# niessner/BundleFusion

Hardware: AMD Instinct MI355X
Metric: frames/sec end-to-end (SIFT+SBA+TSDF re-integrate), 640x480 @4mm (higher is better)
Workload: dtype f32

## Files before the change

bundlefusion_amd/capi.py:

```python
import ctypes as C
import os

import numpy as np

_HERE = os.path.dirname(os.path.abspath(__file__))
LIB_PATH = os.environ.get("BF_LIB_PATH") or os.path.join(_HERE, "lib", "libbf_hip.so")


class BFError(RuntimeError):
    pass


if not os.path.exists(LIB_PATH):
    raise ImportError(
        "bundlefusion_amd: %s is missing — build it with `python -c 'import __graft_entry__ as g; g.build()'` "
        "(there is no CPU fallback)" % LIB_PATH)

try:
    import torch
except ImportError:
    pass
lib = C.CDLL(LIB_PATH, mode=C.RTLD_GLOBAL)

SDF_BLOCK_SIZE = 8
# ... 171 lines not shown
    def set_external_alloc(self, enable=True):
        check(lib.bf_scene_set_external_alloc(self._h, int(enable)))

    def set_alloc_comm(self, comm, capacity_keys=1 << 17):
        check(lib.bf_scene_set_alloc_comm(self._h, comm._h if comm is not None else None, int(capacity_keys)))
        self._alloc_comm = comm

    def alloc_collect(self, cam_to_world, depth, cam, part, parts, keys, slots, count):
        d = self._data(depth, None)
        check(lib.bf_scene_alloc_collect(self._h, mat16(cam_to_world), C.byref(d), C.byref(cam), int(part), int(parts), C.c_void_p(keys.data_ptr()),
                                         C.c_void_p(slots.data_ptr()), C.c_void_p(count.data_ptr()), int(keys.numel())))

    def alloc_ingest(self, keys, count):
        check(lib.bf_scene_alloc_ingest(self._h, C.c_void_p(keys.data_ptr()), C.c_void_p(count.data_ptr()), int(keys.numel())))

    def alloc_place(self):
        check(lib.bf_scene_alloc_place(self._h))

    def alloc_sync(self):
        check(lib.bf_scene_alloc_sync(self._h))

    def set_arith(self, mode):
        check(lib.bf_scene_set_arith(self._h, {"exact": 0, "fast": 1}[mode]))

    def arith(self):
        m = C.c_int()
        check(lib.bf_scene_get_arith(self._h, C.byref(m)))
        return ("exact", "fast")[m.value]

    def reintegrate(self, old_cam_to_world, new_cam_to_world, depth, color, cam):
        data = self._data(depth, color)
        check(lib.bf_scene_reintegrate(self._h, mat16(old_cam_to_world), mat16(new_cam_to_world), C.byref(data), C.byref(cam)))

    def run_batch(self, ops, cam):
        assert 1 <= len(ops) <= SCENE_BATCH_MAX
        arr = (SceneBatchOp * len(ops))()
        for o, (kind, T0, T1, depth, color) in zip(arr, ops):
            o.kind = {"in": 0, "de": 1, "re": 2}.get(kind, kind)
            o.T0[:] = np.asarray(T0, np.float32).reshape(16).tolist()
            o.T1[:] = np.asarray(T1 if T1 is not None else T0, np.float32).reshape(16).tolist()
            o.data = self._data(depth, color)
            o.d_texels = None; o.wait_event = None
        check(lib.bf_scene_run_batch(self._h, arr, len(ops), C.byref(cam)))

    def garbage_collect(self):
        check(lib.bf_scene_garbage_collect(self._h))

    def compactify(self, cam_to_world, cam):
        check(lib.bf_scene_set_last_rigid_transform_and_compactify(self._h, mat16(cam_to_world), C.byref(cam)))

    def hash_data(self):
        hd = HashData()
        check(lib.bf_scene_get_hash_data(self._h, C.byref(hd)))
        return hd

    def hash_params(self):
        p = HashParams()
        check(lib.bf_scene_get_hash_params(self._h, C.byref(p)))
        return p

    def heap_free_count(self):
        v = C.c_uint32()
        check(lib.bf_scene_get_heap_free_count(self._h, C.byref(v)))
        return v.value

    def num_allocated_blocks(self):
        v = C.c_uint32()
        check(lib.bf_scene_get_num_allocated_blocks(self._h, C.byref(v)))
        return v.value

    def num_integrated_frames(self):
        v = C.c_uint32()
        check(lib.bf_scene_get_num_integrated_frames(self._h, C.byref(v)))
        return v.value

    def debug_hash(self):
# ... 1264 lines not shown
```

bundlefusion_amd/csrc/host.hip:

```cpp
#include <algorithm>
#include <atomic>
#include <cmath>
#include <condition_variable>
#include <cstring>
#include <deque>
#include <fstream>
#include <limits>
#include <list>
#include <mutex>
#include <thread>
#include <chrono>
#include <vector>

#include "../../include/bf_pipeline.h"
#include "../../include/bf_comm.h"
#include "../../include/bf_sensordata.h"
#include "bf_device.h"
#include "bf_internal.h"
#include "bf_se3.h"

using namespace bf;

#define BF_TRY(expr) do { int _rc = (expr); if (_rc != BF_OK) return _rc; } while (0)

// ... 1942 lines not shown
    struct VolCmd { int kind; bf_depth_camera_data data; const void* texels; float T0[16], T1[16]; int waitEv; };
    bool volBatching = true;
    std::vector<VolCmd> volPending;
    static const size_t MAX_QUEUE = 48;
    std::thread worker;
    std::mutex mu;
    std::condition_variable cvWork, cvIdle;
    std::deque<VolCmd> queue;
    bool stop = false, busy = false;
    int workerError = BF_OK;
    std::string workerMessage;
    uint32_t numIntegrate = 0, numDeIntegrate = 0;
    double volBusy = 0.0, volCommands = 0.0;
    double hostProfile[8] = {0, 0, 0, 0, 0, 0, 0, 0};
    struct TraceRec { uint32_t frame; double hEnq0, hEnq1, hDet0, hDet1, hWait0, hWait1, hBody1; hipEvent_t gDet, gChain0, gChain1; };
    std::string tracePath; std::vector<TraceRec> trace; hipEvent_t traceBase = nullptr; double traceBaseHost = 0.0;
    TraceRec* traceOf(uint32_t frame) { for (size_t i = trace.size(); i-- > 0;) if (trace[i].frame == frame) return &trace[i]; return nullptr; }
    bool timings = false;
    hipEvent_t ev[10] = {nullptr, nullptr, nullptr, nullptr, nullptr, nullptr, nullptr, nullptr, nullptr, nullptr};
    bf_frame_timing last;
};

namespace {

int volExecute(bf_pipeline* p, const bf_pipeline::VolCmd& c) {
    if (c.kind == 3) return bf_scene_garbage_collect(p->scene);
    if (c.waitEv >= 0) BF_TRY(bf_scene_wait_event(p->scene, p->evIngest[c.waitEv]));
    if (c.texels) BF_TRY(bf_scene_set_frame_texels(p->scene, c.texels));
    if (c.kind == 0) return bf_scene_integrate(p->scene, c.T0, &c.data, &p->cam, nullptr);
    if (c.kind == 1) return bf_scene_deintegrate(p->scene, c.T0, &c.data, &p->cam, nullptr);
    return bf_scene_reintegrate(p->scene, c.T0, c.T1, &c.data, &p->cam);
}

int volSubmitPending(bf_pipeline* p) {
    std::vector<bf_pipeline::VolCmd>& q = p->volPending;
    if (q.empty()) return BF_OK;
    bf_scene_batch_op ops[BF_SCENE_BATCH_MAX];
    const uint32_t n = (uint32_t)q.size();
    for (uint32_t k = 0; k < n; ++k) {
        const bf_pipeline::VolCmd& c = q[k];
        ops[k].kind = c.kind; ops[k].reserved = 0;
        memcpy(ops[k].T0, c.T0, 64); memcpy(ops[k].T1, c.kind == 2 ? c.T1 : c.T0, 64);
        ops[k].data = c.data; ops[k].d_texels = c.texels;
        ops[k].wait_event = c.waitEv >= 0 ? (void*)p->evIngest[c.waitEv] : nullptr;
    }
    q.clear();
    return bf_scene_run_batch(p->scene, ops, n, &p->cam);
}

int volHandle(bf_pipeline* p, const bf_pipeline::VolCmd& c) {
    if (!p->volBatching) return c.kind == 4 ? BF_OK : volExecute(p, c);
    if (c.kind <= 2) {
        p->volPending.push_back(c);
        return p->volPending.size() == BF_SCENE_BATCH_MAX ? volSubmitPending(p) : BF_OK;
    }
    BF_TRY(volSubmitPending(p));
    return c.kind == 3 ? bf_scene_garbage_collect(p->scene) : BF_OK;
}

void volWorker(bf_pipeline* p) {
    for (;;) {
        bf_pipeline::VolCmd c;
        {
            std::unique_lock<std::mutex> lk(p->mu);
            p->cvWork.wait(lk, [p] { return p->stop || !p->queue.empty(); });
            if (p->queue.empty()) return;
            c = p->queue.front(); p->queue.pop_front();
            p->busy = true;
        }
        const double tv = std::chrono::duration<double>(std::chrono::steady_clock::now().time_since_epoch()).count();
        const int rc = volHandle(p, c);
        const double dv = std::chrono::duration<double>(std::chrono::steady_clock::now().time_since_epoch()).count() - tv;
        {
            std::lock_guard<std::mutex> lk(p->mu);
            p->volBusy += dv; p->volCommands += 1.0;
            if (rc != BF_OK && p->workerError == BF_OK) { p->workerError = rc; p->workerMessage = bf_last_error(); }
            p->busy = false;
            p->cvIdle.notify_all();
        }
    }
}

int volPost(bf_pipeline* p, int kind, uint32_t frame, const float* T0, const float* T1, int waitEv) {
    bf_pipeline::VolCmd c;
    c.kind = kind; c.waitEv = waitEv;
    c.data.d_depthData = nullptr; c.data.d_colorData = nullptr;
    c.texels = nullptr;
    if (kind < 3) {
        BF_TRY(bf_image_manager_get_integrate_frame_gpu(p->im, frame, &c.data.d_depthData, &c.data.d_colorData));
        BF_TRY(bf_image_manager_get_integrate_frame_texels(p->im, frame, &c.texels));
// ... 666 lines not shown
```

bundlefusion_amd/csrc/tsdf.hip:

```cpp
#include <hip/hip_runtime.h>

#include <algorithm>
#include <cmath>
#include <cstdlib>
#include <cstring>
#include <strings.h>
#include <unordered_map>
#include <unordered_set>
#include <vector>

#include "bf_device.h"
#include "bf_internal.h"
#include "../../include/bf_comm.h"

using namespace bf;

namespace {

constexpr int BS = BF_SDF_BLOCK_SIZE;
constexpr int VOX = BS * BS * BS;
constexpr uint32_t NBINS = 256;
constexpr uint32_t BINCAP = 4096;
constexpr uint32_t OVCAP = 4096;
constexpr uint32_t TILE = 1024;
// ... 743 lines not shown
        lastFlag = ticket == gridDim.x - 1 ? 1u : 0u;
        if (lastFlag) __builtin_amdgcn_fence(__ATOMIC_ACQUIRE, "agent");
    }
    __syncthreads();
    if (!lastFlag) return;
    placeTail<LISTS>(d, f, fo, s, tailIn[0], tailIn[1], tailIn[2], tailIn[3]);
    if (threadIdx.x == 0) d.stats[ST_TICKET] = 0;
}

__global__ __launch_bounds__(256) void k_compact_count(Dev d) {
    __shared__ uint32_t wsum[4];
    __builtin_amdgcn_s_setprio(3);
    const uint32_t n = d.allocCount[0];
    const uint32_t numTiles = (n + TILE - 1) / TILE;
    for (uint32_t tile = blockIdx.x; tile < numTiles; tile += gridDim.x) {
        uint32_t c = 0;
#pragma unroll
        for (uint32_t k = 0; k < 4; ++k) {
            const uint32_t i = tile * TILE + threadIdx.x * 4 + k;
            if (i < n) c += d.allocList[i].ptr != BF_FREE_ENTRY ? 1u : 0u;
        }
        c = (uint32_t)wave_sum_i((int)c);
        if ((threadIdx.x & 63) == 0) wsum[threadIdx.x >> 6] = c;
        __syncthreads();
        if (threadIdx.x == 0) d.tileCounts[tile] = wsum[0] + wsum[1] + wsum[2] + wsum[3];
        __syncthreads();
    }
}

__global__ __launch_bounds__(256) void k_compact_scatter(Dev d) {
    __shared__ uint32_t wsum[4];
    __builtin_amdgcn_s_setprio(3);
    __shared__ uint32_t wscan[4];
    const uint32_t n = d.allocCount[0];
    const uint32_t numTiles = (n + TILE - 1) / TILE;
    const uint32_t lane = threadIdx.x & 63, wave = threadIdx.x >> 6;
    for (uint32_t tile = blockIdx.x; tile < numTiles; tile += gridDim.x) {
        uint32_t v = 0;
        for (uint32_t t = threadIdx.x; t < tile; t += blockDim.x) v += d.tileCounts[t];
        v = (uint32_t)wave_sum_i((int)v);
        if (lane == 0) wsum[wave] = v;
        __syncthreads();
        const uint32_t base = wsum[0] + wsum[1] + wsum[2] + wsum[3];
        __syncthreads();
        AllocRec recs[4];
        bool keep[4];
        uint32_t c = 0;
#pragma unroll
        for (uint32_t k = 0; k < 4; ++k) {
            const uint32_t i = tile * TILE + threadIdx.x * 4 + k;
            keep[k] = false;
            if (i < n) { recs[k] = d.allocList[i]; keep[k] = recs[k].ptr != BF_FREE_ENTRY; }
            c += keep[k] ? 1u : 0u;
        }
        uint32_t incl = c;
#pragma unroll
        for (int o = 1; o < 64; o <<= 1) { const uint32_t t = __shfl_up(incl, o, 64); if ((int)lane >= o) incl += t; }
        if (lane == 63) wscan[wave] = incl;
        __syncthreads();
        uint32_t woff = 0;
        for (uint32_t w = 0; w < wave; ++w) woff += wscan[w];
        const uint32_t tileTotal = wscan[0] + wscan[1] + wscan[2] + wscan[3];
        uint32_t pos = base + woff + incl - c;
#pragma unroll
        for (uint32_t k = 0; k < 4; ++k) if (keep[k]) d.allocListAlt[pos++] = recs[k];
        if (tile == numTiles - 1 && threadIdx.x == 0) d.tileCounts[numTiles] = base + tileTotal;
        __syncthreads();
    }
}

template <int MODE>
__global__ __launch_bounds__(256) void k_compact_append(Dev d, Frame f, Frame fo) {
    __shared__ uint32_t wscan[4];
    __shared__ uint32_t sbase;
    __builtin_amdgcn_s_setprio(3);
    listAppendTiles<MODE, 4>(d, f, fo, d.allocSnap[0], blockIdx.x, gridDim.x, wscan, &sbase);
}

__global__ void k_alloc_snapshot(Dev d) { d.allocSnap[0] = d.allocCount[0]; d.compactCount[0] = 0; d.compactCount[1] = 0; }

__global__ void k_list_commit(Dev d) {
    const uint32_t n = d.allocCount[0];
    const uint32_t numTiles = (n + TILE - 1) / TILE;
    if (numTiles > 0) d.allocCount[0] = d.tileCounts[numTiles];
}

template <bool DEINT, class FR>
BF_DEV void voxelApply(const FR& f, float sdf, uchar4 cc, float& vSdf, float& vW, uint32_t& vC) {
    const float c0 = (float)cc.x, c1 = (float)cc.y, c2 = (float)cc.z;
    const float oSdf = vSdf, oW = vW;
    const uint32_t oC = vC;
    const float o0 = (float)(oC & 0xFF), o1 = (float)((oC >> 8) & 0xFF), o2 = (float)((oC >> 16) & 0xFF);
    float nSdf, nW;
    uint32_t nC;
    if (!DEINT) {
        float r0, r1, r2;
        if (oW == 0.0f) { r0 = c0; r1 = c1; r2 = c2; }
        else { r0 = 0.2f * c0 + 0.8f * o0; r1 = 0.2f * c1 + 0.8f * o1; r2 = 0.2f * c2 + 0.8f * o2; }
        r0 = fmaxf(0.0f, fminf(__builtin_rintf(r0), 254.5f));
        r1 = fmaxf(0.0f, fminf(__builtin_rintf(r1), 254.5f));
        r2 = fmaxf(0.0f, fminf(__builtin_rintf(r2), 254.5f));
        nC = (uint32_t)(int)r0 | ((uint32_t)(int)r1 << 8) | ((uint32_t)(int)r2 << 16) | 0xFF000000u;
        nSdf = (sdf * 1.0f + oSdf * oW) / (1.0f + oW);
        nW = fminf(f.weightMax, 1.0f + oW);
    } else {
        float r0 = (o0 * oW - c0 * 1.0f) / (oW - 1.0f);
        float r1 = (o1 * oW - c1 * 1.0f) / (oW - 1.0f);
        float r2 = (o2 * oW - c2 * 1.0f) / (oW - 1.0f);
        r0 = fmaxf(0.0f, fminf(roundf(r0), 254.5f));
        r1 = fmaxf(0.0f, fminf(roundf(r1), 254.5f));
        r2 = fmaxf(0.0f, fminf(roundf(r2), 254.5f));
        nC = (uint32_t)(int)r0 | ((uint32_t)(int)r1 << 8) | ((uint32_t)(int)r2 << 16) | 0xFF000000u;
        nSdf = (oSdf * oW - sdf * 1.0f) / (oW - 1.0f);
        nW = fmaxf(0.0f, oW - 1.0f);
        if (nW <= 0.001f) { nSdf = 0.0f; nC = 0u; nW = 0.0f; }
    }
    vSdf = nSdf; vW = nW; vC = nC;
}
// ... 513 lines not shown
                h4[(size_t)i * 2] = h4[(size_t)next * 2];
                h4[(size_t)i * 2 + 1] = h4[(size_t)next * 2 + 1];
                h4[(size_t)next * 2] = make_uint4(0, 0, 0, (uint32_t)BF_FREE_ENTRY);
                h4[(size_t)next * 2 + 1] = make_uint4(0, 0, 0, 0);
            } else {
                h4[(size_t)i * 2] = make_uint4(0, 0, 0, (uint32_t)BF_FREE_ENTRY);
                h4[(size_t)i * 2 + 1] = make_uint4(0, 0, 0, 0);
            }
            return c.ptr;
        }
    }
    const uint32_t last = hp + BF_HASH_BUCKET_SIZE - 1;
    bf_hash_entry c = d.hash[last];
    uint32_t prev = last;
    uint32_t i = (last + c.offset) % total;
    for (uint32_t it = 0; it < f.maxChain; ++it) {
        c = d.hash[i];
        if (c.pos[0] == b.x && c.pos[1] == b.y && c.pos[2] == b.z && c.ptr != BF_FREE_ENTRY) {
            h4[(size_t)i * 2] = make_uint4(0, 0, 0, (uint32_t)BF_FREE_ENTRY);
            h4[(size_t)i * 2 + 1] = make_uint4(0, 0, 0, 0);
            d.hash[prev].offset = c.offset;
            return c.ptr;
        }
        if (c.offset == 0) return BF_FREE_ENTRY;
        prev = i;
        i = (last + c.offset) % total;
    }
    return BF_FREE_ENTRY;
}

__global__ __launch_bounds__(1024) void k_gc_delete(Dev d, Frame f) {
    __shared__ SortLds s;
    __shared__ uint32_t scratch[16];
    const uint32_t bin = blockIdx.x;
    const uint32_t n = min(d.binCount[bin], BINCAP);
    if (n == 0) return;
    loadBinSorted(s, d.bins + (size_t)bin * BINCAP, n);
    const uint32_t base = binPrefix(d.binCount, bin, scratch);
    const uint32_t heapC = d.heapCounter[0];
    for (uint32_t idx = threadIdx.x; idx < n; idx += blockDim.x) {
        const uint32_t h = s.bucket[idx];
        if (idx > 0 && s.bucket[idx - 1] == h) continue;
        for (uint32_t k = idx; k < n && s.bucket[k] == h; ++k) {
            const int32_t ptr = deleteEntry(d, f, unpackKey(s.key[k]), h);
            d.allocList[s.aux[k]].ptr = BF_FREE_ENTRY;
            if (ptr == BF_FREE_ENTRY) { atomicOr(&d.stats[ST_ERROR], (uint32_t)ERR_GC_MISSING); s.aux[k] = 0xFFFFFFFFu; continue; }
            d.heap[heapC + 1u + base + k] = (uint32_t)ptr / (uint32_t)VOX;
            s.aux[k] = (uint32_t)ptr;
        }
    }
    __syncthreads();
    for (uint32_t k = 0; k < n; ++k) {
        const uint32_t ptr = s.aux[k];
        if (ptr == 0xFFFFFFFFu) continue;
        uint4* v4 = reinterpret_cast<uint4*>(d.vox + (size_t)ptr);
        for (uint32_t t = threadIdx.x; t < (uint32_t)(VOX * 12 / 16); t += blockDim.x) v4[t] = make_uint4(0, 0, 0, 0);
    }
}

__global__ __launch_bounds__(256) void k_gc_finish(Dev d) {
    __shared__ uint32_t scratch[16];
    const uint32_t D = binPrefix(d.binCount, NBINS, scratch);
    if (threadIdx.x == 0) d.heapCounter[0] += D;
    __syncthreads();
    for (uint32_t b = threadIdx.x; b < NBINS; b += blockDim.x) d.binCount[b] = 0;
}

}

struct bf_scene {
    bf_hash_params params;
    bf_depth_camera_params cam;
    bool haveCam = false;
    Dev d{};
    hipStream_t stream = nullptr;
    uint32_t numIntegrated = 0;
    uint32_t dedupeSize = 0;
    uint32_t gridCompact = 0, gridUpdateCol = 0, gridUpdateColPlain = 0;
    bool forceExactDiv = false;
    bool externalAlloc = false;
    bf_comm* allocComm = nullptr;
    uint32_t allocCap = 0;
    uint8_t *d_allocSend = nullptr, *d_allocRecv = nullptr; uint32_t* d_allocSlots = nullptr;
    uint8_t *d_batchSend = nullptr, *d_batchRecv = nullptr;
    int arith = BF_TSDF_ARITH_FAST;
    int cvtRne = -1;
    uint2* texel[8] = {}; size_t texelPixels = 0;
    int32_t* d_hashDecision = nullptr;
    uint32_t shardLo = 0, shardHi = 0xFFFFFFFFu;
    uint32_t opsTimed = 0;
    uint32_t imagesTimed = 0;
    bool overlap = false;
    hipStream_t prep = nullptr;
    static constexpr int NBMAX = 8;
    int NB = 4;
    bf_hash_entry* cbuf[NBMAX] = {}; uint32_t* csrc[NBMAX] = {}; int32_t* ccnt[NBMAX] = {};
    int cur = 0;
// ... 419 lines not shown
        auto update = [&](const Dev& dd, int accumulate) {
            if (s->cvtRne) hipLaunchKernelGGL((k_update_batch_apx<true>), dim3(s->gridUpdateCol), dim3(256), s->updateLds, s->stream, dd, ac, ua, accumulate);
            else hipLaunchKernelGGL((k_update_batch_apx<false>), dim3(s->gridUpdateCol), dim3(256), s->updateLds, s->stream, dd, ac, ua, accumulate);
        };
        if (s->verifyPath) {
            BF_TRY_RC(verifyBuffers(s));
            hipLaunchKernelGGL(k_verify_copy, dim3(s->gridUpdateCol), dim3(256), 0, s->stream, dv, s->vshadow[0], s->vshadow[1]);
        }
        update(dv, acc);
        if (s->verifyPath) {
            for (int q = 0; q < 2; ++q) { Dev dq = dv; dq.vox = s->vshadow[q]; update(dq, 0); }
            hipLaunchKernelGGL(k_verify_compare, dim3(s->gridUpdateCol), dim3(256), 0, s->stream, dv, s->vshadow[0], s->vshadow[1], s->vlog, s->vseq++, n, s->gridUpdateCol * 4u);
        }
    } else {
        BatchUpdColArgs ua;
        memset(&ua, 0, sizeof ua);
        ua.nOps = n;
        for (uint32_t k = 0; k < n; ++k) {
            ua.op[k].in = makeUpdPose(fin[k]); ua.op[k].de = makeUpdPose(fde[k]);
            ua.op[k].depth = ops[k].data.d_depthData; ua.op[k].color = reinterpret_cast<const uchar4*>(ops[k].data.d_colorData);
        }
        hipLaunchKernelGGL(k_update_batch_col, dim3(s->gridUpdateCol), dim3(256), 0, s->stream, dv, makeUpdCam(fl), ua, acc, s->forceExactDiv ? 1 : 0);
    }
    if (ev) BF_HIP_TRY(hipEventRecord(ev->second, s->stream));
    if (s->overlap) { BF_HIP_TRY(hipEventRecord(s->evUpd[b], s->stream)); s->updRecorded[b] = true; }
    BF_HIP_TRY(hipGetLastError());
    useBuf(s, b);
    s->compactStale = true;
    s->gcMask = (ops[n - 1].kind == 1 ? 2u : 1u) << (2u * (n - 1));
    for (uint32_t k = 0; k < n; ++k) s->numIntegrated += ops[k].kind == 0 ? 1u : ops[k].kind == 1 ? (uint32_t)-1 : 0u;
    return BF_OK;
}

int checkCall(bf_scene* s, const float* T, const bf_depth_camera_data* data, const bf_depth_camera_params* cam,
              const uint32_t* d_bitMask) {
    BF_REQUIRE(s && T && data && cam, "null argument");
    BF_REQUIRE(data->d_depthData, "d_depthData is null");
    BF_REQUIRE(d_bitMask == nullptr, "chunk streaming (d_bitMask) is not supported: it is disabled for BundleFusion");
    BF_REQUIRE(cam->m_imageWidth > 0 && cam->m_imageHeight > 0, "empty image");
    return BF_OK;
}

}

extern "C" {

int bf_scene_create(const bf_hash_params* p, bf_scene** out) {
    BF_REQUIRE(p && out, "null argument");
    BF_REQUIRE(p->m_hashNumBuckets > 0 && p->m_numSDFBlocks > 0, "empty hash / heap");
    BF_REQUIRE(p->m_hashBucketSize == BF_HASH_BUCKET_SIZE, "m_hashBucketSize must be 4 (HASH_BUCKET_SIZE)");
    BF_REQUIRE(p->m_SDFBlockSize == BF_SDF_BLOCK_SIZE, "m_SDFBlockSize must be 8 (SDF_BLOCK_SIZE)");
    BF_REQUIRE((uint64_t)p->m_hashNumBuckets * BF_HASH_BUCKET_SIZE < 0x7FFFFFFFull, "hash too large for 32-bit slot indices");
    BF_REQUIRE((uint64_t)p->m_numSDFBlocks * VOX < 0x7FFFFFFFull, "too many SDF blocks for the reference's int ptr");
    int ndev = 0;
    if (hipGetDeviceCount(&ndev) != hipSuccess || ndev == 0) { set_error("no HIP device visible"); return BF_ERR_NO_DEVICE; }
    bf_scene* s = new bf_scene();
    s->params = *p;
    const size_t numEntries = (size_t)p->m_hashNumBuckets * BF_HASH_BUCKET_SIZE;
    const size_t N = p->m_numSDFBlocks;
    uint32_t ds = 1u << 16;
    while (ds < 2u * NBINS * BINCAP && ds < 4u * N) ds <<= 1;
    s->dedupeSize = ds;
    int rc = BF_OK;
#define A(ptr, cnt) if (rc == BF_OK) rc = devAlloc(s, &(ptr), (cnt))
    A(s->d.hash, numEntries);
    A(s->d.heap, N);
// ... 228 lines not shown
    int rc = checkCall(s, T, data, cam, d_bitMask);
    if (rc) return rc;
    s->cam = *cam; s->haveCam = true;
    setLastRigidTransform(s, T);
    const Frame f = makeFrame(s);
    if ((rc = runOperator(s, 1, f, f, data))) return rc;
    s->numIntegrated--;
    return BF_OK;
}

int bf_scene_set_shard(bf_scene* s, uint32_t rank, uint32_t world) {
    BF_REQUIRE(s && world >= 1 && rank < world, "bad shard");
    BF_REQUIRE(s->numIntegrated == 0, "set the shard before the first integration");
    const uint64_t nb = s->params.m_hashNumBuckets;
    s->shardLo = (uint32_t)(nb * rank / world);
    s->shardHi = (uint32_t)(nb * (rank + 1) / world);
    return BF_OK;
}

int bf_scene_reintegrate(bf_scene* s, const float oldT[16], const float newT[16], const bf_depth_camera_data* data,
                         const bf_depth_camera_params* cam) {
    int rc = checkCall(s, newT, data, cam, nullptr);
    if (rc) return rc;
    BF_REQUIRE(oldT, "null argument");
    s->cam = *cam; s->haveCam = true;
    setLastRigidTransform(s, oldT);
    const Frame fo = makeFrame(s);
    setLastRigidTransform(s, newT);
    const Frame f = makeFrame(s);
    return runOperator(s, 2, f, fo, data);
}

int bf_scene_run_batch(bf_scene* s, const bf_scene_batch_op* ops, uint32_t n, const bf_depth_camera_params* cam) {
    BF_REQUIRE(s && ops && cam, "null argument");
    BF_REQUIRE(n >= 1 && n <= BF_SCENE_BATCH_MAX, "1 .. BF_SCENE_BATCH_MAX operators per batch");
    BF_REQUIRE(cam->m_imageWidth > 0 && cam->m_imageHeight > 0, "empty image");
    for (uint32_t k = 0; k < n; ++k) {
        BF_REQUIRE(ops[k].kind >= 0 && ops[k].kind <= 2, "unknown operator kind");
        BF_REQUIRE(ops[k].data.d_depthData, "d_depthData is null");
    }
    s->cam = *cam; s->haveCam = true;
    return runBatch(s, ops, n);
}

int bf_scene_set_last_rigid_transform_and_compactify(bf_scene* s, const float T[16], const bf_depth_camera_params* cam) {
    BF_REQUIRE(s && T && cam, "null argument");
    s->cam = *cam; s->haveCam = true;
    setLastRigidTransform(s, T);
    BF_TRY_RC(beginExclusive(s));
    BF_TRY_RC(launchCompactify(s));
    return endExclusive(s);
}

int bf_scene_garbage_collect(bf_scene* s) {
    BF_REQUIRE(s, "null scene");
    if (!s->haveCam) return BF_OK;
    BF_TRY_RC(beginExclusive(s));
    uint32_t needMask = 0;
    if (s->compactStale) { if (s->gcMask) needMask = s->gcMask; else BF_TRY_RC(launchCompactify(s)); }
    const Frame f = makeFrame(s);
    hipLaunchKernelGGL(k_gc_identify, dim3(4096), dim3(256), 0, s->stream, s->d, f, needMask);
    hipLaunchKernelGGL(k_gc_delete, dim3(NBINS), dim3(1024), 0, s->stream, s->d, f);
    hipLaunchKernelGGL(k_gc_finish, dim3(1), dim3(256), 0, s->stream, s->d);
    hipLaunchKernelGGL(k_compact_count, dim3(s->gridCompact), dim3(256), 0, s->stream, s->d);
    hipLaunchKernelGGL(k_compact_scatter, dim3(s->gridCompact), dim3(256), 0, s->stream, s->d);
    hipLaunchKernelGGL(k_list_commit, dim3(1), dim3(1), 0, s->stream, s->d);
    std::swap(s->d.allocList, s->d.allocListAlt);
    BF_HIP_TRY(hipGetLastError());
    s->compactStale = true; s->gcMask = 0;
    return endExclusive(s);
}

int bf_scene_get_hash_data(bf_scene* s, bf_hash_data* out) {
    BF_REQUIRE(s && out, "null argument");
    BF_TRY_RC(refreshStaleList(s));
    BF_TRY_RC(syncAll(s));
    out->d_heap = s->d.heap;
    out->d_heapCounter = s->d.heapCounter;
    out->d_hashDecision = s->d_hashDecision;
    out->d_hashDecisionPrefix = nullptr;
    out->d_hash = s->d.hash;
    out->d_hashCompactified = s->d.compact;
    out->d_hashCompactifiedCounter = s->d.compactCount;
    out->d_SDFBlocks = s->d.vox;
    out->d_hashBucketMutex = nullptr;
    return BF_OK;
}

static int checkDeviceErrors(bf_scene* s) {
    uint32_t stats[ST_COUNT];
    BF_HIP_TRY(hipMemcpyAsync(stats, s->d.stats, sizeof stats, hipMemcpyDeviceToHost, s->stream));
    BF_HIP_TRY(hipStreamSynchronize(s->stream));
    if (stats[ST_ERROR]) { set_error("TSDF scratch capacity exceeded during an earlier operator (error bits 0x%x: 1 bin, 2 de-dup set, 4 overflow list, 8 GC, 16 block list)", stats[ST_ERROR]); return BF_ERR_CAPACITY; }
    return BF_OK;
}

int bf_scene_get_hash_params(bf_scene* s, bf_hash_params* out) {
    BF_REQUIRE(s && out, "null argument");
    BF_TRY_RC(refreshStaleList(s));
    BF_TRY_RC(syncAll(s));
    int32_t n = 0;
    BF_HIP_TRY(hipMemcpyAsync(&n, s->d.compactCount, 4, hipMemcpyDeviceToHost, s->stream));
    BF_HIP_TRY(hipStreamSynchronize(s->stream));
// ... 151 lines not shown
```

include/bf_hip.h:

```cpp
#ifndef BF_HIP_H
#define BF_HIP_H

#include <stddef.h>
#include <stdint.h>

#ifdef __cplusplus
extern "C" {
#endif

#define BF_API __attribute__((visibility("default")))

typedef enum bf_status {
    BF_OK = 0,
    BF_ERR_INVALID_ARG = -1,
    BF_ERR_HIP = -2,
    BF_ERR_NO_DEVICE = -3,
    BF_ERR_CAPACITY = -4,
    BF_ERR_STATE = -5,
    BF_ERR_NOT_ON_DEVICE = -6
} bf_status;

BF_API const char* bf_last_error(void);
BF_API const char* bf_version(void);
BF_API int bf_device_count(void);
// ... 78 lines not shown
                              const bf_depth_camera_data* data,
                              const bf_depth_camera_params* cam, const uint32_t* d_bitMask);
BF_API int bf_scene_deintegrate(bf_scene* s, const float cam_to_world[16],
                                const bf_depth_camera_data* data,
                                const bf_depth_camera_params* cam, const uint32_t* d_bitMask);
BF_API int bf_scene_set_overlap(bf_scene* s, int enable);
BF_API int bf_scene_wait_event(bf_scene* s, void* hip_event);
BF_API int bf_scene_set_shard(bf_scene* s, uint32_t rank, uint32_t world);
BF_API int bf_scene_set_external_alloc(bf_scene* s, int enable);
BF_API int bf_scene_alloc_collect(bf_scene* s, const float cam_to_world[16], const bf_depth_camera_data* data, const bf_depth_camera_params* cam,
                                  uint32_t part, uint32_t parts, uint64_t* d_keys, uint32_t* d_slots, uint32_t* d_count, uint32_t capacity);
BF_API int bf_scene_alloc_ingest(bf_scene* s, const uint64_t* d_keys, const uint32_t* d_count, uint32_t capacity);
BF_API int bf_scene_alloc_place(bf_scene* s);
BF_API int bf_scene_alloc_sync(bf_scene* s);
#define BF_TSDF_ARITH_EXACT 0
#define BF_TSDF_ARITH_FAST 1
BF_API int bf_scene_set_arith(bf_scene* s, int mode);
BF_API int bf_scene_set_frame_texels(bf_scene* s, const void* d_texels);
BF_API int bf_image_interleave_texels(void* d_texels, const float* d_depth, const uint8_t* d_colorRGBX, uint32_t numPixels, void* hip_stream);
BF_API int bf_scene_get_arith(bf_scene* s, int* mode);
BF_API int bf_scene_reintegrate(bf_scene* s, const float old_cam_to_world[16], const float new_cam_to_world[16],
                                const bf_depth_camera_data* data, const bf_depth_camera_params* cam);
#define BF_SCENE_BATCH_MAX 12
typedef struct bf_scene_batch_op {
    int32_t kind;
    int32_t reserved;
    float T0[16], T1[16];
    bf_depth_camera_data data;
    const void* d_texels;
    void* wait_event;
} bf_scene_batch_op;
BF_API int bf_scene_run_batch(bf_scene* s, const bf_scene_batch_op* ops, uint32_t n, const bf_depth_camera_params* cam);
BF_API int bf_scene_garbage_collect(bf_scene* s);
BF_API int bf_scene_set_last_rigid_transform_and_compactify(
    bf_scene* s, const float cam_to_world[16], const bf_depth_camera_params* cam);
BF_API int bf_scene_set_last_rigid_transform(bf_scene* s, const float cam_to_world[16]);
BF_API int bf_scene_get_hash_data(bf_scene* s, bf_hash_data* out);
BF_API int bf_scene_get_hash_params(bf_scene* s, bf_hash_params* out);
BF_API int bf_scene_get_heap_free_count(bf_scene* s, uint32_t* out);
BF_API int bf_scene_get_num_integrated_frames(bf_scene* s, uint32_t* out);
BF_API int bf_scene_debug_hash(bf_scene* s, uint32_t out[6]);
BF_API int bf_scene_debug_find_blocks(bf_scene* s, const int32_t* d_pos, uint32_t n, int32_t* d_ptr_out);
BF_API int bf_scene_get_num_allocated_blocks(bf_scene* s, uint32_t* out);
BF_API int bf_scene_kernel_timing(bf_scene* s, int enable);
BF_API int bf_scene_kernel_timing_read(bf_scene* s, uint32_t* count, float* total_ms);
BF_API int bf_scene_kernel_timing_occupied(bf_scene* s, uint64_t* sumOccupiedBlocks, uint32_t* numOps);
BF_API int bf_scene_kernel_timing_images(bf_scene* s, uint32_t* numImages);
BF_API int bf_scene_kernel_timing_blocks(bf_scene* s, uint64_t* sumOperatorBlocks, uint64_t* visitedPlain, uint64_t* visitedFused, uint32_t* numOps);



typedef struct bf_cached_frame {
    float* d_depthDownsampled;
    float* d_cameraposDownsampled;
    float* d_intensityDownsampled;
    float* d_intensityDerivsDownsampled;
    uint8_t* d_normalsDownsampledUCHAR4;
    float* d_normalsDownsampled;
} bf_cached_frame;

typedef struct bf_cache bf_cache;

BF_API int bf_cache_create(uint32_t widthDepthInput, uint32_t heightDepthInput, uint32_t widthDownSampled,
                           uint32_t heightDownSampled, uint32_t maxNumImages, const float inputIntrinsics[16],
                           float colorDownSigma, float depthDownSigmaD, float depthDownSigmaR, bf_cache** out);
BF_API int bf_cache_destroy(bf_cache* c);
// ... 275 lines not shown
```

include/bundlefusion/bundlefusion.hpp:

```cpp
#pragma once
#include <algorithm>
#include <array>
#include <cstdint>
#include <cstdio>
#include <cmath>
#include <cstring>
#include <fstream>
#include <iostream>
#include <limits>
#include <mutex>
#include <stdexcept>
#include <string>
#include <utility>
#include <vector>

#include "../bf_pipeline.h"
#include "../bf_sensordata.h"

namespace bundlefusion {

struct mat4f {
    float m[16];
    static mat4f identity() { mat4f r; for (int i = 0; i < 16; ++i) r.m[i] = (i % 5 == 0) ? 1.0f : 0.0f; return r; }
    float& operator()(int r, int c) { return m[r * 4 + c]; }
// ... 645 lines not shown
    bf_depth_camera_data d;
};

class CUDASceneRepHashSDF {
public:
    explicit CUDASceneRepHashSDF(const HashParams& params) { check(bf_scene_create(&params, &m_h)); }
    ~CUDASceneRepHashSDF() { try { flush(); } catch (...) {} bf_scene_destroy(m_h); }
    CUDASceneRepHashSDF(const CUDASceneRepHashSDF&) = delete;
    static HashParams parametersFromGlobalAppState(const GlobalAppState& gas) {
        HashParams p;
        std::memset(&p, 0, sizeof p);
        const mat4f I = mat4f::identity();
        std::memcpy(p.m_rigidTransform, I.m, 64); std::memcpy(p.m_rigidTransformInverse, I.m, 64);
        p.m_hashNumBuckets = gas.s_hashNumBuckets; p.m_hashBucketSize = 4; p.m_hashMaxCollisionLinkedListSize = gas.s_hashMaxCollisionLinkedListSize;
        p.m_SDFBlockSize = 8; p.m_numSDFBlocks = gas.s_hashNumSDFBlocks; p.m_virtualVoxelSize = gas.s_SDFVoxelSize;
        p.m_maxIntegrationDistance = gas.s_SDFMaxIntegrationDistance; p.m_truncation = gas.s_SDFTruncation; p.m_truncScale = gas.s_SDFTruncationScale;
        p.m_integrationWeightSample = gas.s_SDFIntegrationWeightSample; p.m_integrationWeightMax = gas.s_SDFIntegrationWeightMax;
        for (int i = 0; i < 3; ++i) { p.m_streamingVoxelExtents[i] = gas.s_streamingVoxelExtents[i]; p.m_streamingGridDimensions[i] = gas.s_streamingGridDimensions[i]; p.m_streamingMinGridPos[i] = gas.s_streamingMinGridPos[i]; }
        p.m_streamingInitialChunkListSize = gas.s_streamingInitialChunkListSize;
        return p;
    }
    void integrate(const mat4f& lastRigidTransform, const DepthCameraData& data, const DepthCameraParams& params, unsigned int* d_bitMask) {
        if (!m_deferred || d_bitMask) { flush(); check(bf_scene_integrate(m_h, lastRigidTransform.m, &data.d, &params, d_bitMask)); return; }
        if (!m_pending.empty() && m_pending.back().kind == 1 && m_pending.back().data.d_depthData == data.d.d_depthData && m_pending.back().data.d_colorData == data.d.d_colorData && m_lastWasDe) {
            m_pending.back().kind = 2; std::memcpy(m_pending.back().T1, lastRigidTransform.m, 64); m_lastWasDe = false;
        } else push(0, lastRigidTransform, data);
        m_cam = params;
    }
    void deIntegrate(const mat4f& lastRigidTransform, const DepthCameraData& data, const DepthCameraParams& params, unsigned int* d_bitMask) {
        if (!m_deferred || d_bitMask) { flush(); check(bf_scene_deintegrate(m_h, lastRigidTransform.m, &data.d, &params, d_bitMask)); return; }
        push(1, lastRigidTransform, data); m_lastWasDe = true;
        m_cam = params;
    }
    void garbageCollect() { flush(); check(bf_scene_garbage_collect(m_h)); }
    void reset() { m_pending.clear(); check(bf_scene_reset(m_h)); }
    void setLastRigidTransformAndCompactify(const mat4f& lastRigidTransform, const DepthCameraParams& params) {
        flush(); check(bf_scene_set_last_rigid_transform_and_compactify(m_h, lastRigidTransform.m, &params));
    }
    void setLastRigidTransform(const mat4f& lastRigidTransform) { flush(); check(bf_scene_set_last_rigid_transform(m_h, lastRigidTransform.m)); }
    const mat4f getLastRigidTransform() { const HashParams p = getHashParams(); mat4f m; std::memcpy(m.m, p.m_rigidTransform, 64); return m; }
    void debugHash() {
        flush();
        uint32_t v[6]; check(bf_scene_debug_hash(m_h, v));
        std::printf("number of occupied entries: %u\nfree heap: %u\nduplicate keys: %u\nallocated and free: %u\nleaked blocks: %u\ndropped: %u\n", v[0], v[1], v[2], v[3], v[4], v[5]);
    }
    HashDataStruct getHashData() { flush(); HashDataStruct d; check(bf_scene_get_hash_data(m_h, &d)); return d; }
    HashParams getHashParams() { flush(); HashParams p; check(bf_scene_get_hash_params(m_h, &p)); return p; }
    unsigned int getHeapFreeCount() { flush(); uint32_t n; check(bf_scene_get_heap_free_count(m_h, &n)); return n; }
    unsigned int getNumIntegratedFrames() { flush(); uint32_t n; check(bf_scene_get_num_integrated_frames(m_h, &n)); return n; }
    bf_scene* handle() const { return m_h; }

    void setDeferredBatching(bool enable) { flush(); m_deferred = enable; }
    void flush() {
        if (m_pending.empty()) return;
        std::vector<bf_scene_batch_op> ops; ops.swap(m_pending);
        m_lastWasDe = false;
        check(bf_scene_run_batch(m_h, ops.data(), (uint32_t)ops.size(), &m_cam));
    }
private:
    void push(int kind, const mat4f& T, const DepthCameraData& data) {
        if (m_pending.size() == BF_SCENE_BATCH_MAX) flush();
        bf_scene_batch_op o; std::memset(&o, 0, sizeof o);
        o.kind = kind; std::memcpy(o.T0, T.m, 64); std::memcpy(o.T1, T.m, 64); o.data = data.d;
        m_pending.push_back(o); m_lastWasDe = false;
    }
    bf_scene* m_h = nullptr;
    bool m_deferred = false, m_lastWasDe = false;
    std::vector<bf_scene_batch_op> m_pending;
    DepthCameraParams m_cam;
};

typedef bf_marching_cubes_params MarchingCubesParams;
typedef bf_ray_cast_params RayCastParams;
typedef bf_ray_cast_data RayCastData;
struct vec3f { float x, y, z; vec3f(float a = 0.0f, float b = 0.0f, float c = 0.0f) : x(a), y(b), z(c) {} };

class CUDAMarchingCubesHashSDF {
public:
    explicit CUDAMarchingCubesHashSDF(const MarchingCubesParams& params) : m_params(params) { check(bf_marching_cubes_create(&params, &m_h)); }
    ~CUDAMarchingCubesHashSDF() { bf_marching_cubes_destroy(m_h); }
    CUDAMarchingCubesHashSDF(const CUDAMarchingCubesHashSDF&) = delete;
    static MarchingCubesParams parametersFromGlobalAppState(const GlobalAppState& gas, unsigned int marchingCubesMaxNumTriangles = 3000000, float SDFMarchingCubeThreshFactor = 10.0f) {
        MarchingCubesParams p;
        p.m_maxNumTriangles = marchingCubesMaxNumTriangles;
        p.m_threshMarchingCubes = SDFMarchingCubeThreshFactor * gas.s_SDFVoxelSize;
        p.m_threshMarchingCubes2 = SDFMarchingCubeThreshFactor * gas.s_SDFVoxelSize;
        p.m_sdfBlockSize = 8; p.m_hashBucketSize = 4; p.m_hashNumBuckets = gas.s_hashNumBuckets;
        return p;
    }
    void clearMeshBuffer() { check(bf_marching_cubes_clear_mesh_buffer(m_h)); }
// ... 49 lines not shown
```

Measured before the change: 1318.

## Fold GC finish and list commit into last-block epilogues; fuse batch with GC

Removes the single-block k_gc_finish and k_list_commit kernels. Their work now runs in a last-block-done epilogue of k_gc_delete and k_compact_scatter, using an atomic ticket counter and an acquire fence. Also adds bf_scene_run_batch_gc so a pending batch and the following garbage collection go through one exclusive API call instead of two. The aim is to cut kernel launches and host API round trips per GC. The cost is an extra atomic and memory wait in every block, plus reliance on the ticket counter being reset correctly.

```diff
diff --git a/bundlefusion_amd/capi.py b/bundlefusion_amd/capi.py
--- a/bundlefusion_amd/capi.py
+++ b/bundlefusion_amd/capi.py
@@ -227,7 +227,7 @@
         data = self._data(depth, color)
         check(lib.bf_scene_reintegrate(self._h, mat16(old_cam_to_world), mat16(new_cam_to_world), C.byref(data), C.byref(cam)))
 
-    def run_batch(self, ops, cam):
+    def run_batch(self, ops, cam, gc=False):
         assert 1 <= len(ops) <= SCENE_BATCH_MAX
         arr = (SceneBatchOp * len(ops))()
         for o, (kind, T0, T1, depth, color) in zip(arr, ops):
@@ -236,7 +236,7 @@
             o.T1[:] = np.asarray(T1 if T1 is not None else T0, np.float32).reshape(16).tolist()
             o.data = self._data(depth, color)
             o.d_texels = None; o.wait_event = None
-        check(lib.bf_scene_run_batch(self._h, arr, len(ops), C.byref(cam)))
+        check((lib.bf_scene_run_batch_gc if gc else lib.bf_scene_run_batch)(self._h, arr, len(ops), C.byref(cam)))
 
     def garbage_collect(self):
         check(lib.bf_scene_garbage_collect(self._h))
diff --git a/bundlefusion_amd/csrc/host.hip b/bundlefusion_amd/csrc/host.hip
--- a/bundlefusion_amd/csrc/host.hip
+++ b/bundlefusion_amd/csrc/host.hip
@@ -1998,9 +1998,9 @@
     return bf_scene_reintegrate(p->scene, c.T0, c.T1, &c.data, &p->cam);
 }
 
-int volSubmitPending(bf_pipeline* p) {
+int volSubmitPending(bf_pipeline* p, bool gc = false) {
     std::vector<bf_pipeline::VolCmd>& q = p->volPending;
-    if (q.empty()) return BF_OK;
+    if (q.empty()) return gc ? bf_scene_garbage_collect(p->scene) : BF_OK;
     bf_scene_batch_op ops[BF_SCENE_BATCH_MAX];
     const uint32_t n = (uint32_t)q.size();
     for (uint32_t k = 0; k < n; ++k) {
@@ -2011,7 +2011,7 @@
         ops[k].wait_event = c.waitEv >= 0 ? (void*)p->evIngest[c.waitEv] : nullptr;
     }
     q.clear();
-    return bf_scene_run_batch(p->scene, ops, n, &p->cam);
+    return gc ? bf_scene_run_batch_gc(p->scene, ops, n, &p->cam) : bf_scene_run_batch(p->scene, ops, n, &p->cam);
 }
 
 int volHandle(bf_pipeline* p, const bf_pipeline::VolCmd& c) {
@@ -2020,8 +2020,7 @@
         p->volPending.push_back(c);
         return p->volPending.size() == BF_SCENE_BATCH_MAX ? volSubmitPending(p) : BF_OK;
     }
-    BF_TRY(volSubmitPending(p));
-    return c.kind == 3 ? bf_scene_garbage_collect(p->scene) : BF_OK;
+    return volSubmitPending(p, c.kind == 3);
 }
 
 void volWorker(bf_pipeline* p) {
diff --git a/bundlefusion_amd/csrc/tsdf.hip b/bundlefusion_amd/csrc/tsdf.hip
--- a/bundlefusion_amd/csrc/tsdf.hip
+++ b/bundlefusion_amd/csrc/tsdf.hip
@@ -799,6 +799,7 @@
     __shared__ uint32_t wsum[4];
     __builtin_amdgcn_s_setprio(3);
     __shared__ uint32_t wscan[4];
+    __shared__ uint32_t lastFlag;
     const uint32_t n = d.allocCount[0];
     const uint32_t numTiles = (n + TILE - 1) / TILE;
     const uint32_t lane = threadIdx.x & 63, wave = threadIdx.x >> 6;
@@ -827,12 +828,28 @@
         __syncthreads();
         uint32_t woff = 0;
         for (uint32_t w = 0; w < wave; ++w) woff += wscan[w];
-        const uint32_t tileTotal = wscan[0] + wscan[1] + wscan[2] + wscan[3];
         uint32_t pos = base + woff + incl - c;
 #pragma unroll
         for (uint32_t k = 0; k < 4; ++k) if (keep[k]) d.allocListAlt[pos++] = recs[k];
-        if (tile == numTiles - 1 && threadIdx.x == 0) d.tileCounts[numTiles] = base + tileTotal;
         __syncthreads();
+    }
+    asm volatile("s_waitcnt vmcnt(0)" ::: "memory");
+    __syncthreads();
+    if (threadIdx.x == 0) {
+        const uint32_t ticket = atomicAdd(&d.stats[ST_TICKET], 1u);
+        lastFlag = ticket == gridDim.x - 1 ? 1u : 0u;
+        if (lastFlag) __builtin_amdgcn_fence(__ATOMIC_ACQUIRE, "agent");
+    }
+    __syncthreads();
+    if (!lastFlag) return;
+    uint32_t v = 0;
+    for (uint32_t t = threadIdx.x; t < numTiles; t += blockDim.x) v += d.tileCounts[t];
+    v = (uint32_t)wave_sum_i((int)v);
+    if (lane == 0) wsum[wave] = v;
+    __syncthreads();
+    if (threadIdx.x == 0) {
+        if (numTiles > 0) d.allocCount[0] = wsum[0] + wsum[1] + wsum[2] + wsum[3];
+        d.stats[ST_TICKET] = 0;
     }
 }
 
@@ -845,12 +862,6 @@
 }
 
 __global__ void k_alloc_snapshot(Dev d) { d.allocSnap[0] = d.allocCount[0]; d.compactCount[0] = 0; d.compactCount[1] = 0; }
-
-__global__ void k_list_commit(Dev d) {
-    const uint32_t n = d.allocCount[0];
-    const uint32_t numTiles = (n + TILE - 1) / TILE;
-    if (numTiles > 0) d.allocCount[0] = d.tileCounts[numTiles];
-}
 
 template <bool DEINT, class FR>
 BF_DEV void voxelApply(const FR& f, float sdf, uchar4 cc, float& vSdf, float& vW, uint32_t& vC) {
@@ -1430,37 +1441,43 @@
 __global__ __launch_bounds__(1024) void k_gc_delete(Dev d, Frame f) {
     __shared__ SortLds s;
     __shared__ uint32_t scratch[16];
+    __shared__ uint32_t lastFlag;
     const uint32_t bin = blockIdx.x;
     const uint32_t n = min(d.binCount[bin], BINCAP);
-    if (n == 0) return;
-    loadBinSorted(s, d.bins + (size_t)bin * BINCAP, n);
-    const uint32_t base = binPrefix(d.binCount, bin, scratch);
-    const uint32_t heapC = d.heapCounter[0];
-    for (uint32_t idx = threadIdx.x; idx < n; idx += blockDim.x) {
-        const uint32_t h = s.bucket[idx];
-        if (idx > 0 && s.bucket[idx - 1] == h) continue;
-        for (uint32_t k = idx; k < n && s.bucket[k] == h; ++k) {
-            const int32_t ptr = deleteEntry(d, f, unpackKey(s.key[k]), h);
-            d.allocList[s.aux[k]].ptr = BF_FREE_ENTRY;
-            if (ptr == BF_FREE_ENTRY) { atomicOr(&d.stats[ST_ERROR], (uint32_t)ERR_GC_MISSING); s.aux[k] = 0xFFFFFFFFu; continue; }
-            d.heap[heapC + 1u + base + k] = (uint32_t)ptr / (uint32_t)VOX;
-            s.aux[k] = (uint32_t)ptr;
-        }
-    }
+    if (n != 0) {
+        loadBinSorted(s, d.bins + (size_t)bin * BINCAP, n);
+        const uint32_t base = binPrefix(d.binCount, bin, scratch);
+        const uint32_t heapC = d.heapCounter[0];
+        for (uint32_t idx = threadIdx.x; idx < n; idx += blockDim.x) {
+            const uint32_t h = s.bucket[idx];
+            if (idx > 0 && s.bucket[idx - 1] == h) continue;
+            for (uint32_t k = idx; k < n && s.bucket[k] == h; ++k) {
+                const int32_t ptr = deleteEntry(d, f, unpackKey(s.key[k]), h);
+                d.allocList[s.aux[k]].ptr = BF_FREE_ENTRY;
+                if (ptr == BF_FREE_ENTRY) { atomicOr(&d.stats[ST_ERROR], (uint32_t)ERR_GC_MISSING); s.aux[k] = 0xFFFFFFFFu; continue; }
+                d.heap[heapC + 1u + base + k] = (uint32_t)ptr / (uint32_t)VOX;
+                s.aux[k] = (uint32_t)ptr;
+            }
+        }
+        __syncthreads();
+        for (uint32_t k = 0; k < n; ++k) {
+            const uint32_t ptr = s.aux[k];
+            if (ptr == 0xFFFFFFFFu) continue;
+            uint4* v4 = reinterpret_cast<uint4*>(d.vox + (size_t)ptr);
+            for (uint32_t t = threadIdx.x; t < (uint32_t)(VOX * 12 / 16); t += blockDim.x) v4[t] = make_uint4(0, 0, 0, 0);
+        }
+    }
+    asm volatile("s_waitcnt vmcnt(0)" ::: "memory");
     __syncthreads();
-    for (uint32_t k = 0; k < n; ++k) {
-        const uint32_t ptr = s.aux[k];
-        if (ptr == 0xFFFFFFFFu) continue;
-        uint4* v4 = reinterpret_cast<uint4*>(d.vox + (size_t)ptr);
-        for (uint32_t t = threadIdx.x; t < (uint32_t)(VOX * 12 / 16); t += blockDim.x) v4[t] = make_uint4(0, 0, 0, 0);
-    }
-}
-
-__global__ __launch_bounds__(256) void k_gc_finish(Dev d) {
-    __shared__ uint32_t scratch[16];
+    if (threadIdx.x == 0) {
+        const uint32_t ticket = atomicAdd(&d.stats[ST_TICKET], 1u);
+        lastFlag = ticket == gridDim.x - 1 ? 1u : 0u;
+        if (lastFlag) __builtin_amdgcn_fence(__ATOMIC_ACQUIRE, "agent");
+    }
+    __syncthreads();
+    if (!lastFlag) return;
     const uint32_t D = binPrefix(d.binCount, NBINS, scratch);
-    if (threadIdx.x == 0) d.heapCounter[0] += D;
-    __syncthreads();
+    if (threadIdx.x == 0) { d.heapCounter[0] += D; d.stats[ST_TICKET] = 0; }
     for (uint32_t b = threadIdx.x; b < NBINS; b += blockDim.x) d.binCount[b] = 0;
 }
 
@@ -1946,6 +1963,32 @@
     return BF_OK;
 }
 
+int checkBatch(bf_scene* s, const bf_scene_batch_op* ops, uint32_t n, const bf_depth_camera_params* cam) {
+    BF_REQUIRE(s && ops && cam, "null argument");
+    BF_REQUIRE(n >= 1 && n <= BF_SCENE_BATCH_MAX, "1 .. BF_SCENE_BATCH_MAX operators per batch");
+    BF_REQUIRE(cam->m_imageWidth > 0 && cam->m_imageHeight > 0, "empty image");
+    for (uint32_t k = 0; k < n; ++k) {
+        BF_REQUIRE(ops[k].kind >= 0 && ops[k].kind <= 2, "unknown operator kind");
+        BF_REQUIRE(ops[k].data.d_depthData, "d_depthData is null");
+    }
+    return BF_OK;
+}
+
+int collectGarbage(bf_scene* s) {
+    BF_TRY_RC(beginExclusive(s));
+    uint32_t needMask = 0;
+    if (s->compactStale) { if (s->gcMask) needMask = s->gcMask; else BF_TRY_RC(launchCompactify(s)); }
+    const Frame f = makeFrame(s);
+    hipLaunchKernelGGL(k_gc_identify, dim3(4096), dim3(256), 0, s->stream, s->d, f, needMask);
+    hipLaunchKernelGGL(k_gc_delete, dim3(NBINS), dim3(1024), 0, s->stream, s->d, f);
+    hipLaunchKernelGGL(k_compact_count, dim3(s->gridCompact), dim3(256), 0, s->stream, s->d);
+    hipLaunchKernelGGL(k_compact_scatter, dim3(s->gridCompact), dim3(256), 0, s->stream, s->d);
+    std::swap(s->d.allocList, s->d.allocListAlt);
+    BF_HIP_TRY(hipGetLastError());
+    s->compactStale = true; s->gcMask = 0;
+    return endExclusive(s);
+}
+
 int checkCall(bf_scene* s, const float* T, const bf_depth_camera_data* data, const bf_depth_camera_params* cam,
               const uint32_t* d_bitMask) {
     BF_REQUIRE(s && T && data && cam, "null argument");
@@ -2240,15 +2283,16 @@
 }
 
 int bf_scene_run_batch(bf_scene* s, const bf_scene_batch_op* ops, uint32_t n, const bf_depth_camera_params* cam) {
-    BF_REQUIRE(s && ops && cam, "null argument");
-    BF_REQUIRE(n >= 1 && n <= BF_SCENE_BATCH_MAX, "1 .. BF_SCENE_BATCH_MAX operators per batch");
-    BF_REQUIRE(cam->m_imageWidth > 0 && cam->m_imageHeight > 0, "empty image");
-    for (uint32_t k = 0; k < n; ++k) {
-        BF_REQUIRE(ops[k].kind >= 0 && ops[k].kind <= 2, "unknown operator kind");
-        BF_REQUIRE(ops[k].data.d_depthData, "d_depthData is null");
-    }
+    BF_TRY_RC(checkBatch(s, ops, n, cam));
     s->cam = *cam; s->haveCam = true;
     return runBatch(s, ops, n);
+}
+
+int bf_scene_run_batch_gc(bf_scene* s, const bf_scene_batch_op* ops, uint32_t n, const bf_depth_camera_params* cam) {
+    BF_TRY_RC(checkBatch(s, ops, n, cam));
+    s->cam = *cam; s->haveCam = true;
+    BF_TRY_RC(runBatch(s, ops, n));
+    return collectGarbage(s);
 }
 
 int bf_scene_set_last_rigid_transform_and_compactify(bf_scene* s, const float T[16], const bf_depth_camera_params* cam) {
@@ -2263,20 +2307,7 @@
 int bf_scene_garbage_collect(bf_scene* s) {
     BF_REQUIRE(s, "null scene");
     if (!s->haveCam) return BF_OK;
-    BF_TRY_RC(beginExclusive(s));
-    uint32_t needMask = 0;
-    if (s->compactStale) { if (s->gcMask) needMask = s->gcMask; else BF_TRY_RC(launchCompactify(s)); }
-    const Frame f = makeFrame(s);
-    hipLaunchKernelGGL(k_gc_identify, dim3(4096), dim3(256), 0, s->stream, s->d, f, needMask);
-    hipLaunchKernelGGL(k_gc_delete, dim3(NBINS), dim3(1024), 0, s->stream, s->d, f);
-    hipLaunchKernelGGL(k_gc_finish, dim3(1), dim3(256), 0, s->stream, s->d);
-    hipLaunchKernelGGL(k_compact_count, dim3(s->gridCompact), dim3(256), 0, s->stream, s->d);
-    hipLaunchKernelGGL(k_compact_scatter, dim3(s->gridCompact), dim3(256), 0, s->stream, s->d);
-    hipLaunchKernelGGL(k_list_commit, dim3(1), dim3(1), 0, s->stream, s->d);
-    std::swap(s->d.allocList, s->d.allocListAlt);
-    BF_HIP_TRY(hipGetLastError());
-    s->compactStale = true; s->gcMask = 0;
-    return endExclusive(s);
+    return collectGarbage(s);
 }
 
 int bf_scene_get_hash_data(bf_scene* s, bf_hash_data* out) {
diff --git a/include/bf_hip.h b/include/bf_hip.h
--- a/include/bf_hip.h
+++ b/include/bf_hip.h
@@ -134,6 +134,7 @@
 } bf_scene_batch_op;
 BF_API int bf_scene_run_batch(bf_scene* s, const bf_scene_batch_op* ops, uint32_t n, const bf_depth_camera_params* cam);
 BF_API int bf_scene_garbage_collect(bf_scene* s);
+BF_API int bf_scene_run_batch_gc(bf_scene* s, const bf_scene_batch_op* ops, uint32_t n, const bf_depth_camera_params* cam);
 BF_API int bf_scene_set_last_rigid_transform_and_compactify(
     bf_scene* s, const float cam_to_world[16], const bf_depth_camera_params* cam);
 BF_API int bf_scene_set_last_rigid_transform(bf_scene* s, const float cam_to_world[16]);
diff --git a/include/bundlefusion/bundlefusion.hpp b/include/bundlefusion/bundlefusion.hpp
--- a/include/bundlefusion/bundlefusion.hpp
+++ b/include/bundlefusion/bundlefusion.hpp
@@ -701,7 +701,7 @@
         push(1, lastRigidTransform, data); m_lastWasDe = true;
         m_cam = params;
     }
-    void garbageCollect() { flush(); check(bf_scene_garbage_collect(m_h)); }
+    void garbageCollect() { if (!flush(true)) check(bf_scene_garbage_collect(m_h)); }
     void reset() { m_pending.clear(); check(bf_scene_reset(m_h)); }
     void setLastRigidTransformAndCompactify(const mat4f& lastRigidTransform, const DepthCameraParams& params) {
         flush(); check(bf_scene_set_last_rigid_transform_and_compactify(m_h, lastRigidTransform.m, &params));
@@ -720,11 +720,12 @@
     bf_scene* handle() const { return m_h; }
 
     void setDeferredBatching(bool enable) { flush(); m_deferred = enable; }
-    void flush() {
-        if (m_pending.empty()) return;
+    bool flush(bool gc = false) {
+        if (m_pending.empty()) return false;
         std::vector<bf_scene_batch_op> ops; ops.swap(m_pending);
         m_lastWasDe = false;
-        check(bf_scene_run_batch(m_h, ops.data(), (uint32_t)ops.size(), &m_cam));
+        check(gc ? bf_scene_run_batch_gc(m_h, ops.data(), (uint32_t)ops.size(), &m_cam) : bf_scene_run_batch(m_h, ops.data(), (uint32_t)ops.size(), &m_cam));
+        return gc;
     }
 private:
     void push(int kind, const mat4f& T, const DepthCameraData& data) {
```

Measured after the change: 1306. About the same (-0.9%).
